# KleistLab/WarpDemuX

Hardware: AMD Instinct MI355X
Metric: reads/sec demuxed (110-pt DTW x 10 barcodes) (higher is better)
Workload: dtype f64; 1 GPU; C3: 10000000 synthetic RNA004 adapter reads per GPU (10000000 in all; wdx-synth v1, mean 4665 samples), WDX10 shape: 10 barcodes x 110-pt fingerprints, window 15, penalty 0.1; fused fingerprint+DTW+call+count, raw rows resident in HBM; reads_per_gpu=10000000, reads_total=10000000, failed_reads=0, count_allreduce=none (one process)

## Files before the change

### warpdemux_amd/csrc/wdx_clip.hip

```cpp

#include "wdx_fp_types.h"
#include "wdx_wave.h"

#include <algorithm>
#include <type_traits>

namespace wdx {

typedef float v2f __attribute__((ext_vector_type(2)));

constexpr int kClipWaves = 1;
constexpr int kClipWaveWords = kHB + 64;

struct ClipArgs {
    FpArgs a;
    ClipRec *rec;
    int cap;
    const unsigned *in_count;
    const int32_t *in_list;
    int defer;
};

__device__ __forceinline__ unsigned clip_xor8(unsigned x) { return WDX_DPP(0u, x, 0x128, 0xf); }
__device__ __forceinline__ unsigned clip_xor2(unsigned x) { return WDX_DPP(0u, x, 0x4e, 0xf); }
__device__ __forceinline__ unsigned clip_xor1(unsigned x) { return WDX_DPP(0u, x, 0xb1, 0xf); }
__device__ __forceinline__ unsigned clip_xor4(unsigned x) {
    return (unsigned)__builtin_amdgcn_ds_swizzle((int)x, 0x101f);
}
__device__ __forceinline__ void clip_wave_fence() {
    __builtin_amdgcn_fence(__ATOMIC_ACQ_REL, "wavefront");
    __builtin_amdgcn_wave_barrier();
}

template <int NPL>
__device__ __forceinline__ void clip_wave(const FpArgs &A, ClipRec *recs, const int64_t r, const int cap, unsigned *lds,
                                          const bool defer = false) {
    static_assert(NPL % 4 == 0 && NPL * 64 <= 16384, "samples per lane");
    const int lane = threadIdx.x & 63;
    const wdx_seg_params &P = A.p;
    unsigned *hist = lds;
    unsigned *wl = lds + kHB;

    const int64_t row_off = A.row_off ? A.row_off[r] : r * A.stride;
    const int64_t row_len = A.row_len ? (int64_t)A.row_len[r] : (A.row_off ? A.row_off[r + 1] - A.row_off[r] : A.stride);
    int64_t start = (int64_t)A.a_start[r] - P.padding;
    if (start < 0) start = 0;
    int64_t stop = (int64_t)A.a_end[r] + P.padding;
    if (stop > row_len) stop = row_len;
    const int64_t n64 = stop - start;
    ClipRec out{0.0f, 0.0f, 0.0f, CLIP_NONE};
    if ((A.ok && !A.ok[r]) || n64 < 256 || n64 > (int64_t)cap) {
        if (lane == 0) recs[r] = out;
        return;
    }
    const int n = (int)n64;
    constexpr int NG = NPL / 4;
    const int ng = (n + 255) >> 8;
    long long *pp = (A.prof && r < A.prof_reads) ? A.prof + r * 32 : nullptr;
    auto stamp = [&](int k) __attribute__((always_inline)) {
        if (pp) {
            const long long t = (long long)__builtin_amdgcn_s_memtime();
            if (lane == 0) pp[k] = t;
        }
    };
    stamp(26);

    unsigned u[NPL];
    {
        struct __attribute__((packed, aligned(4))) F4U { unsigned x, y, z, w; };
        const unsigned *__restrict__ src = reinterpret_cast<const unsigned *>(A.sig + row_off + start);
        const unsigned last4 = (unsigned)(n - 4);
#pragma unroll
        for (int j = 0; j < NG; ++j) {
            u[4 * j] = u[4 * j + 1] = u[4 * j + 2] = u[4 * j + 3] = 0u;
            if (j < ng) {
                const unsigned i = (unsigned)(j * 64 + lane) * 4u;
                const F4U v = *reinterpret_cast<const F4U *>(src + min(i, last4));
                u[4 * j] = v.x; u[4 * j + 1] = v.y; u[4 * j + 2] = v.z; u[4 * j + 3] = v.w;
            }
        }
    }
    unsigned umn = 0xffffffffu, umx = 0u;
#pragma unroll
    for (int j = 0; j < NG; ++j) {
        if (j < ng) {
            umn = min(min(umn, u[4 * j]), u[4 * j + 1]);
            umn = min(min(umn, u[4 * j + 2]), u[4 * j + 3]);
            umx = max(max(umx, u[4 * j]), u[4 * j + 1]);
            umx = max(max(umx, u[4 * j + 2]), u[4 * j + 3]);
        }
    }
    umn = wave_min_u32(umn);
    umx = wave_max_u32(umx);
    stamp(27);
    const bool neg = umx > 0x7f800000u;
    float xmin_true = __uint_as_float(umn);
    if (neg) {
        int smx = 0;
#pragma unroll
        for (int j = 0; j < NG; ++j) {
            if (j < ng) {
#pragma unroll
                for (int q = 0; q < 4; ++q) smx = max(smx, (int)u[4 * j + q]);
            }
        }
        smx = (int)wave_max_u32((unsigned)smx);
        if (umx >= 0xff800000u || (unsigned)smx >= 0x7f800000u || umn >= 0x7f800000u) {
            out.flag = defer ? CLIP_NONE : CLIP_NAN_NEG;
            if (lane == 0) recs[r] = out;
            return;
        }
        xmin_true = __uint_as_float(umx);
#pragma unroll
        for (int j = 0; j < NG; ++j) {
            if (j < ng) {
#pragma unroll
                for (int q = 0; q < 4; ++q) u[4 * j + q] = (unsigned)max((int)u[4 * j + q], (int)umn);
            }
        }
        umx = (unsigned)smx;
    } else if (umx >= 0x7f800000u) {
        out.flag = defer ? CLIP_NONE : CLIP_NAN_NEG;
        if (lane == 0) recs[r] = out;
        return;
    }
    const unsigned last4 = (unsigned)(n - 4);
    const unsigned i_last = (unsigned)((ng - 1) * 64 + lane) * 4u;
    auto pad_last_group = [&](unsigned padkey) __attribute__((always_inline)) {
#pragma unroll
        for (int j = 0; j < NG; ++j) {
            if (j == ng - 1) {
#pragma unroll
                for (int q = 0; q < 4; ++q) {
                    const bool valid = min(i_last, last4) + (unsigned)q >= i_last;
                    u[4 * j + q] = valid ? u[4 * j + q] : padkey;
                }
            }
        }
    };
    pad_last_group(umx);

    auto each4 = [&](auto &&f4) __attribute__((always_inline)) {
        int ngp = ng;
        asm volatile("" : "+s"(ngp));
#pragma unroll
        for (int j = 0; j < NG; ++j) {
            if (j < ngp) f4(u[4 * j], u[4 * j + 1], u[4 * j + 2], u[4 * j + 3]);
        }
    };
    auto each = [&](auto &&f) __attribute__((always_inline)) {
        each4([&](unsigned x0, unsigned x1, unsigned x2, unsigned x3) __attribute__((always_inline)) {
            f(x0);
            f(x1);
            f(x2);
            f(x3);
        });
    };

    unsigned sk, sa, sb;
    unsigned klo = 0, khi = 0;
    bool in_hi = false, done = false;
    float med = 0.0f, lin_scale = 0.0f;
    auto level = [&](auto mode_t, auto mad_t) __attribute__((always_inline)) {
        constexpr int MODE = decltype(mode_t)::value;
        constexpr bool MAD = decltype(mad_t)::value;
        const unsigned a = sa, b = sb, k = sk;
        const unsigned range = b - a;
        int shift = 32 - __clz((int)range) - kHBits;
        if (shift < 0) shift = 0;
        if (((b >> shift) - (a >> shift)) >= (unsigned)kHB) ++shift;
        const unsigned abin = a >> shift;
        auto opaque = [](float v) __attribute__((always_inline)) -> float {
            asm volatile("" : "+v"(v));
            return v;
        };
        __builtin_amdgcn_s_setprio(0);
        {
            uint4 *h4 = reinterpret_cast<uint4 *>(hist);
#pragma unroll
            for (int q = 0; q < kHB / 256; ++q) h4[q * 64 + lane] = make_uint4(0, 0, 0, 0);
        }
        clip_wave_fence();
        if constexpr (MODE == 1) {
            const float m1 = opaque(med), s1 = opaque(lin_scale);
            const v2f m1v = {m1, m1}, s1v = {s1, s1};
            each4([&](unsigned x0, unsigned x1, unsigned x2, unsigned x3) __attribute__((always_inline)) {
                const v2f pa = (v2f{__uint_as_float(x0), __uint_as_float(x1)} - m1v) * s1v;
                const v2f pb = (v2f{__uint_as_float(x2), __uint_as_float(x3)} - m1v) * s1v;
                atomicAdd(&hist[(unsigned)fabsf(pa.x)], 1u);
                atomicAdd(&hist[(unsigned)fabsf(pa.y)], 1u);
                atomicAdd(&hist[(unsigned)fabsf(pb.x)], 1u);
                atomicAdd(&hist[(unsigned)fabsf(pb.y)], 1u);
            });
        } else if constexpr (MODE == 0) {
            unsigned *hb = hist - abin;
            each([&](unsigned key) { atomicAdd(&hb[key >> shift], 1u); });
        } else {
            unsigned *hb = hist - abin;
            const float m1 = opaque(med);
            each([&](unsigned x) {
                unsigned key = x;
                if constexpr (MAD) {
                    float d = __uint_as_float(x) - m1;
                    asm("" : "+v"(d));
                    key = __float_as_uint(fabsf(d));
                }
                if (key - a <= range) atomicAdd(&hb[key >> shift], 1u);
            });
        }
        clip_wave_fence();
        __builtin_amdgcn_s_setprio(1);
        if constexpr (MODE == 0) stamp(28);
        if constexpr (MODE == 1) stamp(23);
        unsigned B, cnt, kin;
        {
            const uint2 *h2 = reinterpret_cast<const uint2 *>(hist);
            unsigned s[16];
#pragma unroll
            for (int q = 0; q < 16; ++q) {
                const uint2 v = h2[q * 64 + lane];
                s[q] = v.x + v.y;
            }
#pragma unroll
            for (int q = 0; q < 8; ++q) {
                const auto sw = __builtin_amdgcn_permlane32_swap(s[q], s[q + 8], false, false);
                s[q] = sw[0] + sw[1];
            }
#pragma unroll
            for (int q = 0; q < 4; ++q) {
                const auto sw = __builtin_amdgcn_permlane16_swap(s[q], s[q + 4], false, false);
                s[q] = sw[0] + sw[1];
            }
            const bool b3 = (lane & 8) != 0, b2 = (lane & 4) != 0;
#pragma unroll
            for (int q = 0; q < 2; ++q) {
                const unsigned keep = b3 ? s[q + 2] : s[q], give = b3 ? s[q] : s[q + 2];
                s[q] = keep + clip_xor8(give);
            }
            {
                const unsigned keep = b2 ? s[1] : s[0], give = b2 ? s[0] : s[1];
                s[0] = keep + clip_xor4(give);
            }
            unsigned T = s[0];
            T += clip_xor2(T);
            T += clip_xor1(T);
            const unsigned incl = wave_incl_scan_u32((lane & 3) == 0 ? T : 0u);
            const unsigned long long mk = __ballot(incl > k);
            const int fl = (int)__builtin_ctzll(mk);
            const unsigned qs = (unsigned)fl >> 2;
            const unsigned k2 = k - (unsigned)__builtin_amdgcn_readlane((int)(incl - T), fl);
            const uint2 c = h2[qs * 64 + lane];
            const unsigned ps = c.x + c.y;
            const unsigned incl2 = wave_incl_scan_u32(ps);
            const unsigned long long mk2 = __ballot(incl2 > k2);
            const int l2 = (int)__builtin_ctzll(mk2);
            unsigned k3 = k2 - (unsigned)__builtin_amdgcn_readlane((int)(incl2 - ps), l2);
            const unsigned cx = (unsigned)__builtin_amdgcn_readlane((int)c.x, l2);
            const unsigned cy = (unsigned)__builtin_amdgcn_readlane((int)c.y, l2);
            B = qs * 128u + 2u * (unsigned)l2;
            cnt = cx;
            if (k3 >= cx) {
                k3 -= cx;
                B += 1u;
                cnt = cy;
            }
            kin = k3;
        }
        if constexpr (MODE == 0) stamp(29);
        unsigned ma = a, mspan = 0u;
        if constexpr (MODE != 1) {
            const unsigned lo_b = (B + abin) << shift, hi_b = lo_b + ((1u << shift) - 1u);
            ma = lo_b > a ? lo_b : a;
            mspan = (hi_b < b ? hi_b : b) - ma;
        }
        auto classify = [&](unsigned x, float m2, float s2, unsigned &key) __attribute__((always_inline)) -> bool {
            key = x;
            if constexpr (MAD) {
                float d = __uint_as_float(x) - m2;
                asm("" : "+v"(d));
                key = __float_as_uint(fabsf(d));
                if constexpr (MODE == 1) return (unsigned)fabsf(d * s2) == B;
            }
            return (key - ma) <= mspan;
        };
        if (cnt <= 64u) {
            unsigned wc = 0;
            const float m2 = opaque(med), s2 = opaque(lin_scale);
            auto put = [&](bool mbr, unsigned key) __attribute__((always_inline)) {
                const unsigned long long mask = __ballot(mbr);
                if (mask) {
                    const unsigned at = __builtin_amdgcn_mbcnt_hi((unsigned)(mask >> 32),
                                                                  __builtin_amdgcn_mbcnt_lo((unsigned)mask, 0u));
                    if (mbr) wl[wc + at] = key;
                    wc += (unsigned)__popcll(mask);
                }
            };
            if constexpr (MODE == 1) {
                const v2f m2v = {m2, m2}, s2v = {s2, s2};
                each4([&](unsigned x0, unsigned x1, unsigned x2, unsigned x3) __attribute__((always_inline)) {
                    const v2f da = v2f{__uint_as_float(x0), __uint_as_float(x1)} - m2v, pa = da * s2v;
                    const v2f db = v2f{__uint_as_float(x2), __uint_as_float(x3)} - m2v, pb = db * s2v;
                    put((unsigned)fabsf(pa.x) == B, __float_as_uint(fabsf(da.x)));
                    put((unsigned)fabsf(pa.y) == B, __float_as_uint(fabsf(da.y)));
                    put((unsigned)fabsf(pb.x) == B, __float_as_uint(fabsf(db.x)));
                    put((unsigned)fabsf(pb.y) == B, __float_as_uint(fabsf(db.y)));
                });
            } else {
                each([&](unsigned x) {
                    unsigned key;
                    const bool mbr = classify(x, m2, s2, key);
                    put(mbr, key);
                });
            }
            clip_wave_fence();
            const unsigned mine = (unsigned)lane < cnt ? wl[lane] : 0xffffffffu;
            unsigned rank = 0;
            for (unsigned j = 0; j < cnt; ++j) {
                const unsigned o = (unsigned)__builtin_amdgcn_readlane((int)mine, (int)j);
                rank += (o < mine || (o == mine && j < (unsigned)lane)) ? 1u : 0u;
            }
            const bool mem = (unsigned)lane < cnt;
            klo = (unsigned)__builtin_amdgcn_readlane((int)mine, (int)__builtin_ctzll(__ballot(mem && rank == kin)));
            if (kin + 1u < cnt) {
                khi = (unsigned)__builtin_amdgcn_readlane((int)mine, (int)__builtin_ctzll(__ballot(mem && rank == kin + 1u)));
                in_hi = true;
            }
            done = true;
            return;
        }
        unsigned mmn = 0xffffffffu, mmx = 0u;
        {
            const float m2 = opaque(med), s2 = opaque(lin_scale);
            each([&](unsigned x) {
                unsigned key;
                const bool mbr = classify(x, m2, s2, key);
                mmn = min(mmn, mbr ? key : 0xffffffffu);
                mmx = max(mmx, mbr ? key : 0u);
            });
        }
        sa = wave_min_u32(mmn);
        sb = wave_max_u32(mmx);
        sk = kin;
        if (sa == sb) {
            klo = khi = sa;
            in_hi = kin + 1u < cnt;
            done = true;
        }
    };
    auto select = [&](auto mad_t, unsigned k, unsigned a, unsigned b, unsigned m, const bool want_hi) __attribute__((always_inline)) {
        constexpr bool MAD = decltype(mad_t)::value;
        sk = k; sa = a; sb = b;
        in_hi = false;
        done = false;
        if (a == b) {
            klo = khi = a;
            in_hi = k + 1u < m;
        } else {
            if constexpr (MAD) level(std::integral_constant<int, 1>{}, mad_t);
            else level(std::integral_constant<int, 0>{}, mad_t);
#pragma clang loop unroll(disable)
            while (!done) level(std::integral_constant<int, 2>{}, mad_t);
        }
        if (want_hi && !in_hi) {
            unsigned nxt = 0xffffffffu;
            const unsigned kl = klo;
            float m2 = med;
            asm volatile("" : "+v"(m2));
            each([&](unsigned x) {
                unsigned key = x;
                if constexpr (MAD) {
                    float d = __uint_as_float(x) - m2;
                    asm("" : "+v"(d));
                    key = __float_as_uint(fabsf(d));
                }
                nxt = min(nxt, key > kl ? key : 0xffffffffu);
            });
            khi = wave_min_u32(nxt);
        }
    };

    const unsigned h = (unsigned)n / 2u;
    const bool odd = (n & 1) != 0;
    const unsigned m_all = (unsigned)ng * 256u;
    select(std::false_type{}, odd ? h : h - 1u, umn, umx, m_all, !odd);
    stamp(30);
    if (neg && klo == umn) {
        out.flag = defer ? CLIP_NONE : CLIP_INEXACT;
        if (lane == 0) recs[r] = out;
        return;
    }
    med = odd ? __uint_as_float(klo) : (__uint_as_float(klo) + __uint_as_float(khi)) / 2.0f;
    const float xmin = __uint_as_float(umn), xmax = __uint_as_float(umx);
    const float dmin_ = fabsf(xmin - med), dmax_ = fabsf(xmax - med);
    const float dmax = fmaxf(dmin_, dmax_);
    const unsigned dmaxk = __float_as_uint(dmax);
    pad_last_group(__float_as_uint(dmin_ > dmax_ ? xmin : xmax));
    lin_scale = dmax > 0.0f ? (float)(kHB - 1) / dmax : 1.0f;
    if (!(lin_scale > 0.0f && lin_scale < 3.0e38f)) {
        out.flag = defer ? CLIP_NONE : CLIP_INEXACT;
        if (lane == 0) recs[r] = out;
        return;
    }
    stamp(31);
    select(std::true_type{}, odd ? h : h - 1u, 0u, dmaxk, m_all, !odd);
    stamp(24);
    if (neg && (odd ? klo : khi) >= __float_as_uint(dmin_)) {
        out.flag = defer ? CLIP_NONE : CLIP_INEXACT;
        if (lane == 0) recs[r] = out;
        return;
    }
    const float mad = odd ? __uint_as_float(klo) : (__uint_as_float(klo) + __uint_as_float(khi)) / 2.0f;
    float lo, hi;
    clip_bounds(P, med, mad, lo, hi);
    const float cmin = __builtin_amdgcn_fmed3f(xmin_true, lo, hi);
    const float cmax = __builtin_amdgcn_fmed3f(xmax, lo, hi);
    bool exact = (lo == lo) && (hi == hi) && lo <= hi && cmin > 0.0f && cmax < 3.0e38f;
    if (exact) {
        int fa = (int)(__float_as_uint(cmin) >> 23), fb = (int)(__float_as_uint(cmax) >> 23);
        if (fa == 0) fa = 1;
        exact = (fb - fa) + (32 - __clz(n)) <= 28;
    }
    out.lo = lo;
    out.hi = hi;
    out.cmax = cmax;
    out.flag = exact ? CLIP_OK : CLIP_INEXACT;
    if (lane == 0) recs[r] = out;
}

constexpr int clip_wgs_per_cu(int npl) { return (npl <= 80 ? 4 : (npl <= 128 ? 3 : 2)) * (4 / kClipWaves); }

template <int NPL>
__global__ __launch_bounds__(kClipWaves * 64, clip_wgs_per_cu(NPL)) void clip_bounds_kernel(ClipArgs C) {
    __shared__ __attribute__((aligned(16))) unsigned clip_lds[kClipWaves][kClipWaveWords];
    const int wave = __builtin_amdgcn_readfirstlane((int)(threadIdx.x >> 6));
    const int64_t r = C.a.block_base + (int64_t)blockIdx.x * kClipWaves + wave;
    if (r >= C.a.n_reads) return;
    clip_wave<NPL>(C.a, C.rec, r, C.cap, clip_lds[wave]);
}

template <int NPL>
__global__ __launch_bounds__(kClipWaves * 64, clip_wgs_per_cu(NPL)) void clip_bounds_list_kernel(ClipArgs C) {
    __shared__ __attribute__((aligned(16))) unsigned clip_lds[kClipWaves][kClipWaveWords];
    const int wave = __builtin_amdgcn_readfirstlane((int)(threadIdx.x >> 6));
    const int64_t k = C.a.block_base + (int64_t)blockIdx.x * kClipWaves + wave;
    if (k >= (int64_t)*C.in_count) return;
    const int64_t r = C.in_list[k];
    if (C.rec[r].flag != CLIP_NONE) return;
    clip_wave<NPL>(C.a, C.rec, r, C.cap, clip_lds[wave], C.defer != 0);
}

__global__ __launch_bounds__(1024) void route_long_windows_kernel(FpArgs A, int cap, unsigned *big_count, int32_t *big_list) {
    __shared__ unsigned wcnt[16], wbase;
    const int64_t r = A.block_base + (int64_t)blockIdx.x * 1024 + threadIdx.x;
    const int wave = (int)(threadIdx.x >> 6);
    bool take = false;
    if (r < A.n_reads && !(A.ok && !A.ok[r])) {
        const int64_t row_len = A.row_len ? (int64_t)A.row_len[r] : (A.row_off ? A.row_off[r + 1] - A.row_off[r] : A.stride);
        int64_t start = (int64_t)A.a_start[r] - A.p.padding;
        if (start < 0) start = 0;
        int64_t stop = (int64_t)A.a_end[r] + A.p.padding;
        if (stop > row_len) stop = row_len;
        take = stop - start > (int64_t)cap;
    }
    const unsigned long long mask = __ballot(take);
    if ((threadIdx.x & 63) == 0) wcnt[wave] = (unsigned)__popcll(mask);
    __syncthreads();
    if (threadIdx.x == 0) {
        unsigned tot = 0;
        for (int w = 0; w < 16; ++w) tot += wcnt[w];
        wbase = tot ? atomicAdd(big_count, tot) : 0u;
    }
    __syncthreads();
    if (!take) return;
    unsigned base = wbase;
    for (int w = 0; w < wave; ++w) base += wcnt[w];
    const unsigned at = __builtin_amdgcn_mbcnt_hi((unsigned)(mask >> 32), __builtin_amdgcn_mbcnt_lo((unsigned)mask, 0u));
    big_list[base + at] = (int32_t)r;
}

int launch_route_long_windows(const FpArgs &A, int cap, unsigned *d_count, int32_t *d_list, hipStream_t stream) {
    FpArgs R = A;
    const int64_t n_wg = (A.n_reads + 1023) / 1024, max_slice = launch_slice_limit(1ll << 21);
    for (int64_t base = 0; base < n_wg; base += max_slice) {
        R.block_base = base * 1024;
        hipLaunchKernelGGL(route_long_windows_kernel, dim3((unsigned)std::min<int64_t>(max_slice, n_wg - base)), dim3(1024), 0, stream,
                           R, cap, d_count, d_list);
    }
    WDX_HIP_TRY(hipGetLastError());
    return WDX_SUCCESS;
}

int launch_clip_bounds_list(const FpArgs &A, ClipRec *d_rec, const unsigned *d_count, const int32_t *d_list, int64_t n_entries,
                            hipStream_t stream, int cap, bool defer) {
    if (n_entries <= 0) return WDX_SUCCESS;
    if (cap != 6144 && cap != 8192 && cap != kClipWaveLongCap) {
        set_error("clip_bounds_list_kernel: capacities are 6144, 8192 and 13312 samples");
        return WDX_ERR_INVALID;
    }
    void (*kclip)(ClipArgs) = cap == 6144 ? clip_bounds_list_kernel<96> : (cap == 8192 ? clip_bounds_list_kernel<128> : clip_bounds_list_kernel<kClipWaveLongCap / 64>);
    ClipArgs CA{A, d_rec, cap, d_count, d_list, defer ? 1 : 0};
    const int64_t n_wg = (n_entries + kClipWaves - 1) / kClipWaves, max_slice = launch_slice_limit(1ll << 22);
    for (int64_t base = 0; base < n_wg; base += max_slice) {
        CA.a.block_base = base * kClipWaves;
        hipLaunchKernelGGL(kclip, dim3((unsigned)std::min<int64_t>(max_slice, n_wg - base)), dim3(kClipWaves * 64), 0, stream, CA);
    }
    WDX_HIP_TRY(hipGetLastError());
    return WDX_SUCCESS;
}

int launch_clip_bounds(const FpArgs &A, ClipRec *d_rec, int cap, hipStream_t stream) {
    if (cap > kClipWaveLongCap) {
        set_error("clip_bounds_kernel takes windows of at most 13312 samples");
        return WDX_ERR_INVALID;
    }
    void (*kclip)(ClipArgs) = cap <= 4096 ? clip_bounds_kernel<64> : (cap <= 5120 ? clip_bounds_kernel<80> : (cap <= 6144 ? clip_bounds_kernel<96>
                              : (cap <= 8192 ? clip_bounds_kernel<128> : clip_bounds_kernel<kClipWaveLongCap / 64>)));
    ClipArgs CA{A, d_rec, cap, nullptr, nullptr, 0};
    const int64_t n_wg = (A.n_reads + kClipWaves - 1) / kClipWaves, max_slice = launch_slice_limit(1ll << 22);
    for (int64_t base = 0; base < n_wg; base += max_slice) {
        CA.a.block_base = base * kClipWaves;
        hipLaunchKernelGGL(kclip, dim3((unsigned)std::min<int64_t>(max_slice, n_wg - base)), dim3(kClipWaves * 64), 0, stream, CA);
    }
    WDX_HIP_TRY(hipGetLastError());
    return WDX_SUCCESS;
}

int launch_clip_bounds_selftest(const float *d_sig, const int64_t *d_row_off, int64_t stride, int64_t n_reads,
                                const int32_t *d_a_start, const int32_t *d_a_end, const wdx_seg_params &p, int cap,
                                void *d_rec, hipStream_t stream) {
    FpArgs A{};
    A.sig = d_sig;
    A.row_off = d_row_off;
    A.stride = stride;
    A.n_reads = n_reads;
    A.a_start = d_a_start;
    A.a_end = d_a_end;
    A.p = p;
    return launch_clip_bounds(A, reinterpret_cast<ClipRec *>(d_rec), cap, stream);
}

}
```

Before: 50.74 million reads/s.

## Reduce clip kernel register and LDS pressure to raise occupancy

Shrinks per-wave LDS by aliasing the small selection worklist onto the histogram buffer, with an added fence before reuse. It streams the histogram reduction through nested lambdas so fewer of the 16 partial sums stay live at once, and forces median and scale values into scalar registers. The launch-bounds occupancy hint is changed from a per-CU formula to a waves-per-SIMD table that asks for 5 waves at small NPL. The aim is fewer VGPRs and more resident waves, at the cost of extra LDS round-trips and a possible correctness risk if the worklist aliasing races with histogram reads.

```diff
diff --git a/warpdemux_amd/csrc/wdx_clip.hip b/warpdemux_amd/csrc/wdx_clip.hip
--- a/warpdemux_amd/csrc/wdx_clip.hip
+++ b/warpdemux_amd/csrc/wdx_clip.hip
@@ -10,7 +10,7 @@
 typedef float v2f __attribute__((ext_vector_type(2)));
 
 constexpr int kClipWaves = 1;
-constexpr int kClipWaveWords = kHB + 64;
+constexpr int kClipWaveWords = kHB;
 
 struct ClipArgs {
     FpArgs a;
@@ -27,6 +27,9 @@
 __device__ __forceinline__ unsigned clip_xor4(unsigned x) {
     return (unsigned)__builtin_amdgcn_ds_swizzle((int)x, 0x101f);
 }
+__device__ __forceinline__ float clip_uniform(float v) {
+    return __int_as_float(__builtin_amdgcn_readfirstlane(__float_as_int(v)));
+}
 __device__ __forceinline__ void clip_wave_fence() {
     __builtin_amdgcn_fence(__ATOMIC_ACQ_REL, "wavefront");
     __builtin_amdgcn_wave_barrier();
@@ -39,7 +42,7 @@
     const int lane = threadIdx.x & 63;
     const wdx_seg_params &P = A.p;
     unsigned *hist = lds;
-    unsigned *wl = lds + kHB;
+    unsigned *wl = lds;
 
     const int64_t row_off = A.row_off ? A.row_off[r] : r * A.stride;
     const int64_t row_len = A.row_len ? (int64_t)A.row_len[r] : (A.row_off ? A.row_off[r + 1] - A.row_off[r] : A.stride);
@@ -126,19 +129,27 @@
     }
     const unsigned last4 = (unsigned)(n - 4);
     const unsigned i_last = (unsigned)((ng - 1) * 64 + lane) * 4u;
+    unsigned inv = i_last - min(i_last, last4);
+    asm volatile("" : "+v"(inv));
     auto pad_last_group = [&](unsigned padkey) __attribute__((always_inline)) {
 #pragma unroll
         for (int j = 0; j < NG; ++j) {
             if (j == ng - 1) {
 #pragma unroll
                 for (int q = 0; q < 4; ++q) {
-                    const bool valid = min(i_last, last4) + (unsigned)q >= i_last;
+                    const bool valid = (unsigned)q >= inv;
                     u[4 * j + q] = valid ? u[4 * j + q] : padkey;
                 }
             }
         }
     };
     pad_last_group(umx);
+
+    auto lane_now = [&]() __attribute__((always_inline)) -> int {
+        int l = lane;
+        asm volatile("" : "+v"(l));
+        return l;
+    };
 
     auto each4 = [&](auto &&f4) __attribute__((always_inline)) {
         int ngp = ng;
@@ -176,9 +187,9 @@
         };
         __builtin_amdgcn_s_setprio(0);
         {
-            uint4 *h4 = reinterpret_cast<uint4 *>(hist);
-#pragma unroll
-            for (int q = 0; q < kHB / 256; ++q) h4[q * 64 + lane] = make_uint4(0, 0, 0, 0);
+            uint4 *h4 = reinterpret_cast<uint4 *>(hist) + lane_now();
+#pragma unroll
+            for (int q = 0; q < kHB / 256; ++q) h4[q * 64] = make_uint4(0, 0, 0, 0);
         }
         clip_wave_fence();
         if constexpr (MODE == 1) {
@@ -215,28 +226,31 @@
         unsigned B, cnt, kin;
         {
             const uint2 *h2 = reinterpret_cast<const uint2 *>(hist);
-            unsigned s[16];
-#pragma unroll
-            for (int q = 0; q < 16; ++q) {
-                const uint2 v = h2[q * 64 + lane];
-                s[q] = v.x + v.y;
-            }
-#pragma unroll
-            for (int q = 0; q < 8; ++q) {
-                const auto sw = __builtin_amdgcn_permlane32_swap(s[q], s[q + 8], false, false);
-                s[q] = sw[0] + sw[1];
-            }
-#pragma unroll
-            for (int q = 0; q < 4; ++q) {
-                const auto sw = __builtin_amdgcn_permlane16_swap(s[q], s[q + 4], false, false);
-                s[q] = sw[0] + sw[1];
-            }
+            const uint2 *h2l = h2 + lane_now();
+            auto row = [&](int q) __attribute__((always_inline)) -> unsigned {
+                const uint2 v = h2l[q * 64];
+                return v.x + v.y;
+            };
+            auto half = [&](int q) __attribute__((always_inline)) -> unsigned {
+                const auto sw = __builtin_amdgcn_permlane32_swap(row(q), row(q + 8), false, false);
+                unsigned t = sw[0] + sw[1];
+                asm volatile("" : "+v"(t));
+                return t;
+            };
+            auto quad = [&](int q) __attribute__((always_inline)) -> unsigned {
+                const unsigned x = half(q), y = half(q + 4);
+                const auto sw = __builtin_amdgcn_permlane16_swap(x, y, false, false);
+                return sw[0] + sw[1];
+            };
             const bool b3 = (lane & 8) != 0, b2 = (lane & 4) != 0;
-#pragma unroll
-            for (int q = 0; q < 2; ++q) {
-                const unsigned keep = b3 ? s[q + 2] : s[q], give = b3 ? s[q] : s[q + 2];
-                s[q] = keep + clip_xor8(give);
-            }
+            auto pair = [&](int q) __attribute__((always_inline)) -> unsigned {
+                const unsigned x = quad(q), y = quad(q + 2);
+                const unsigned keep = b3 ? y : x, give = b3 ? x : y;
+                return keep + clip_xor8(give);
+            };
+            unsigned s[2];
+            s[0] = pair(0);
+            s[1] = pair(1);
             {
                 const unsigned keep = b2 ? s[1] : s[0], give = b2 ? s[0] : s[1];
                 s[0] = keep + clip_xor4(give);
@@ -249,7 +263,7 @@
             const int fl = (int)__builtin_ctzll(mk);
             const unsigned qs = (unsigned)fl >> 2;
             const unsigned k2 = k - (unsigned)__builtin_amdgcn_readlane((int)(incl - T), fl);
-            const uint2 c = h2[qs * 64 + lane];
+            const uint2 c = h2l[qs * 64];
             const unsigned ps = c.x + c.y;
             const unsigned incl2 = wave_incl_scan_u32(ps);
             const unsigned long long mk2 = __ballot(incl2 > k2);
@@ -284,6 +298,7 @@
             return (key - ma) <= mspan;
         };
         if (cnt <= 64u) {
+            clip_wave_fence();
             unsigned wc = 0;
             const float m2 = opaque(med), s2 = opaque(lin_scale);
             auto put = [&](bool mbr, unsigned key) __attribute__((always_inline)) {
@@ -313,7 +328,7 @@
                 });
             }
             clip_wave_fence();
-            const unsigned mine = (unsigned)lane < cnt ? wl[lane] : 0xffffffffu;
+            const unsigned mine = (unsigned)lane < cnt ? wl[lane_now()] : 0xffffffffu;
             unsigned rank = 0;
             for (unsigned j = 0; j < cnt; ++j) {
                 const unsigned o = (unsigned)__builtin_amdgcn_readlane((int)mine, (int)j);
@@ -389,13 +404,13 @@
         if (lane == 0) recs[r] = out;
         return;
     }
-    med = odd ? __uint_as_float(klo) : (__uint_as_float(klo) + __uint_as_float(khi)) / 2.0f;
+    med = clip_uniform(odd ? __uint_as_float(klo) : (__uint_as_float(klo) + __uint_as_float(khi)) / 2.0f);
     const float xmin = __uint_as_float(umn), xmax = __uint_as_float(umx);
-    const float dmin_ = fabsf(xmin - med), dmax_ = fabsf(xmax - med);
-    const float dmax = fmaxf(dmin_, dmax_);
+    const float dmin_ = clip_uniform(fabsf(xmin - med)), dmax_ = clip_uniform(fabsf(xmax - med));
+    const float dmax = clip_uniform(fmaxf(dmin_, dmax_));
     const unsigned dmaxk = __float_as_uint(dmax);
     pad_last_group(__float_as_uint(dmin_ > dmax_ ? xmin : xmax));
-    lin_scale = dmax > 0.0f ? (float)(kHB - 1) / dmax : 1.0f;
+    lin_scale = clip_uniform(dmax > 0.0f ? (float)(kHB - 1) / dmax : 1.0f);
     if (!(lin_scale > 0.0f && lin_scale < 3.0e38f)) {
         out.flag = defer ? CLIP_NONE : CLIP_INEXACT;
         if (lane == 0) recs[r] = out;
@@ -427,21 +442,21 @@
     if (lane == 0) recs[r] = out;
 }
 
-constexpr int clip_wgs_per_cu(int npl) { return (npl <= 80 ? 4 : (npl <= 128 ? 3 : 2)) * (4 / kClipWaves); }
+constexpr int clip_waves_per_simd(int npl) { return npl <= 80 ? 5 : (npl <= 96 ? 4 : (npl <= 128 ? 3 : 2)); }
 
 template <int NPL>
-__global__ __launch_bounds__(kClipWaves * 64, clip_wgs_per_cu(NPL)) void clip_bounds_kernel(ClipArgs C) {
+__global__ __launch_bounds__(kClipWaves * 64, clip_waves_per_simd(NPL)) void clip_bounds_kernel(ClipArgs C) {
     __shared__ __attribute__((aligned(16))) unsigned clip_lds[kClipWaves][kClipWaveWords];
-    const int wave = __builtin_amdgcn_readfirstlane((int)(threadIdx.x >> 6));
+    const int wave = kClipWaves == 1 ? 0 : __builtin_amdgcn_readfirstlane((int)(threadIdx.x >> 6));
     const int64_t r = C.a.block_base + (int64_t)blockIdx.x * kClipWaves + wave;
     if (r >= C.a.n_reads) return;
     clip_wave<NPL>(C.a, C.rec, r, C.cap, clip_lds[wave]);
 }
 
 template <int NPL>
-__global__ __launch_bounds__(kClipWaves * 64, clip_wgs_per_cu(NPL)) void clip_bounds_list_kernel(ClipArgs C) {
+__global__ __launch_bounds__(kClipWaves * 64, clip_waves_per_simd(NPL)) void clip_bounds_list_kernel(ClipArgs C) {
     __shared__ __attribute__((aligned(16))) unsigned clip_lds[kClipWaves][kClipWaveWords];
-    const int wave = __builtin_amdgcn_readfirstlane((int)(threadIdx.x >> 6));
+    const int wave = kClipWaves == 1 ? 0 : __builtin_amdgcn_readfirstlane((int)(threadIdx.x >> 6));
     const int64_t k = C.a.block_base + (int64_t)blockIdx.x * kClipWaves + wave;
     if (k >= (int64_t)*C.in_count) return;
     const int64_t r = C.in_list[k];
```

Result: faster. 51.42 million reads/s, median of 6 (+1.3%).
